# andrewcsmith/vox_box.rs

Hardware: AMD Instinct MI355X
Metric: frames/sec (pitch+LPC+formants), 48 kHz 25 ms/10 ms hop, 1→8 MI355X (higher is better)
Workload: dtype f64

## Files before the change

### vox_box.rs_amd/csrc/k_spectral.hip

```cpp
#include "vbx_spectral_1200.hpp"

namespace vbx {

static size_t spectral_lds_bytes(int n) {
    size_t need = (size_t)pitch_refine_lds_bytes(n);
    const size_t t2_end = (size_t)SP_T2_LDS_OFFSET + 60 * sizeof(double2);
    if (t2_end > need) need = t2_end;
    return (need + 15) & ~(size_t)15;
}

int spectral_plan(int n) {
    static const int min_n = [] { const char *e = getenv("VBX_SPECTRAL_MIN_N"); return e ? atoi(e) : SPECTRAL_MIN_N; }();
    if (n < min_n || n < 64) return SPECTRAL_PLAN_NONE;
    if (n <= 1024) return SPECTRAL_PLAN_1024;
    if (n <= SP_N) return SPECTRAL_PLAN_1200;
    if (n <= 2048) return SPECTRAL_PLAN_2048;
    if (n <= 4096) return SPECTRAL_PLAN_4096;
    return SPECTRAL_PLAN_NONE;
}

int spectral_plan_nc(int plan) {
    return plan == SPECTRAL_PLAN_1200 ? SP_N : plan == SPECTRAL_PLAN_1024 ? 1024 : plan == SPECTRAL_PLAN_2048 ? 2048 :
           plan == SPECTRAL_PLAN_4096 ? 4096 : 0;
}

int spectral_tab_complex(int plan) {
    return plan == SPECTRAL_PLAN_1200 ? SPECTRAL_TAB_COMPLEX : spectral_pow2_tab_complex(plan);
}

void spectral_fill_tab(int plan, double *h) {
    if (plan != SPECTRAL_PLAN_1200) { spectral_pow2_fill_tab(plan, h); return; }
    const long double two_pi = 6.283185307179586476925286766559005768L;
    size_t o = 0;
    auto put = [&](long num, long den) {
        const long double ang = two_pi * (long double)(num % den) / (long double)den;
        h[o++] = (double)cosl(ang); h[o++] = (double)(-sinl(ang));
    };
    for (long np = 0; np < 60; np++) for (long ka = 0; ka < 20; ka++) put(np * ka, 1200);
    for (long c = 0; c < 3; c++) for (long kb = 0; kb < 20; kb++) put(c * kb, 60);
    for (long m = 0; m <= 600; m++) put(m, 2400);
}

bool spectral_supported(int n, int lpc_order, int mfcc_nb, int mfcc_b_lo, int num_coeffs) {
    const int plan = spectral_plan(n);
    if (plan == SPECTRAL_PLAN_NONE) return false;
    if (lpc_order != 0 && lpc_order != SP_LPC_P) return false;
    if (num_coeffs != 0 && ((2 * spectral_plan_nc(plan)) % n != 0 || (n & 1) || num_coeffs > 64 || mfcc_nb < 1 || mfcc_b_lo < 0 || mfcc_b_lo + mfcc_nb > n / 2)) return false;
    return true;
}

int spectral_plan_mfcc(int n) {
    const int plan = spectral_plan(n);
    if (plan == SPECTRAL_PLAN_NONE) return plan;
    if ((2 * spectral_plan_nc(plan)) % n == 0) return plan;
    if (n <= SP_N && (2 * SP_N) % n == 0 && !(n & 1)) return SPECTRAL_PLAN_1200;
    return plan;
}
bool spectral_supported_plan(int plan, int n, int lpc_order, int mfcc_nb, int mfcc_b_lo, int num_coeffs) {
    if (plan == SPECTRAL_PLAN_NONE || n > spectral_plan_nc(plan)) return false;
    if (lpc_order != 0 && lpc_order != SP_LPC_P) return false;
    if (num_coeffs != 0 && ((2 * spectral_plan_nc(plan)) % n != 0 || (n & 1) || num_coeffs > 64 || mfcc_nb < 1 || mfcc_b_lo < 0 || mfcc_b_lo + mfcc_nb > n / 2)) return false;
    return true;
}

static void mfcc_interp_geom(int plan, long *M, int *nt, int *lds_cap) {
    *M = 2L * spectral_plan_nc(plan);
    *nt = plan == SPECTRAL_PLAN_4096 ? 128 : 64;
    *lds_cap = (plan == SPECTRAL_PLAN_1200 || plan == SPECTRAL_PLAN_1024) ? (160 * 1024) / 11 : plan == SPECTRAL_PLAN_2048 ? (160 * 1024) / 7 : (160 * 1024) / 4;
}
static int mfcc_interp_slots(int plan, int nb) { long M; int nt, cap; mfcc_interp_geom(plan, &M, &nt, &cap); return (nb + nt - 1) / nt; }

int mfcc_interp_taps(int plan, int n) {
    long M; int nt, cap; mfcc_interp_geom(plan, &M, &nt, &cap);
    const double tau = 0.5 - (double)n / (2.0 * (double)M);
#ifdef VBX_EXP_INTERP_FEWER_TAPS
    return tau >= 0.36 ? 24 : tau >= 0.268 ? 32 : MFCC_INTERP_MAX_TAPS;
#endif
    return tau >= 0.401 ? 24 : tau >= 0.298 ? 32 : MFCC_INTERP_MAX_TAPS;
}

size_t mfcc_interp_table_bytes(int plan, int nb) {
    long M; int nt, cap; mfcc_interp_geom(plan, &M, &nt, &cap);
    const size_t slots = (size_t)mfcc_interp_slots(plan, nb);
    return (size_t)(M / 4 + 1) * 16 + slots * (MFCC_INTERP_MAX_TAPS / 2) * nt * 16 + slots * nt * 4;
}
size_t mfcc_interp_coef_offset(int plan) { return (size_t)(2L * spectral_plan_nc(plan) / 4 + 1) * 16; }
size_t mfcc_interp_j0_offset(int plan, int nb) {
    long M; int nt, cap; mfcc_interp_geom(plan, &M, &nt, &cap);
    return mfcc_interp_coef_offset(plan) + (size_t)mfcc_interp_slots(plan, nb) * (MFCC_INTERP_MAX_TAPS / 2) * nt * 16;
}

// ... 31 lines not shown
        const long first = (i < nb) ? (k * M) / n - W / 2 + 1 : jmin;
        j0t[i] = (int32_t)(first - jmin);
        for (int t = 0; t < W; t++) {
            long double c = 0.0L;
            if (i < nb) {
                const long num = k * M - (first + t) * (long)n;
                if (num == 0) c = 1.0L;
                else {
                    const long double nu = (long double)num / (long double)n;
                    long r = num % (2L * n); if (r < 0) r += 2L * n;
                    const long double sn = sinl(pi * (long double)r / (long double)n);
                    const long double arg = beta * beta - (2.0L * pi * tau * nu) * (2.0L * pi * tau * nu);
                    const long double bump = sinhc(arg > 0.0L ? sqrtl(arg) : 0.0L) / norm;
                    c = sn / (pi * nu) * bump;
                }
            }
            coef[(((size_t)u * HT + t / 2) * NT + th) * 2 + (t & 1)] = (double)c;
        }
    }
    const int zn = (int)(jmax - jmin + 1), nbp = (nb + 1) & ~1;
    d->jmin = (int)jmin; d->jmax = (int)jmax; d->taps = W;
    d->pu_off = 2 * zn;
    d->lds_bytes = (2 * zn + 2 * nbp + 64) * 8;
    d->rot = nullptr; d->coef = nullptr; d->j0 = nullptr;
    return d->lds_bytes <= cap;
}

bool spectral_list_parked(const spectral_launch_t &L) {
    const bool rows16 = (((uintptr_t)L.out_cand) & 15) == 0 && (L.cand_ld & 1) == 0;
    return L.plan == SPECTRAL_PLAN_1200 && pitch_full_list_bytes(L.n, L.kmax) != 0 && L.kmax >= pitch_full_list_entries(L.n) &&
           L.out_r == nullptr && !L.mfcc_only && rows16;
}

int launch_analyze(hipStream_t s, const spectral_launch_t &L) {
    if (L.x.kind != SAMPLE_F64 && (L.plan != SPECTRAL_PLAN_1200 || L.n != SP_N)) return -1;
    spectral_args_t a;
    a.frames = static_cast<const double *>(L.x.p);
    a.n_frames = L.F; a.stride = L.stride; a.window = L.window; a.lag_window = L.lag_window;
    a.tab = reinterpret_cast<const double2 *>(L.tab);
    a.n = L.n;
    a.pp.sample_rate = L.sample_rate; a.pp.threshold = L.threshold; a.pp.fmin = L.fmin; a.pp.fmax = L.fmax; a.pp.kmax = L.kmax; a.pp.f32 = 0;
    a.out_cand = reinterpret_cast<double *>(L.out_cand); a.cand_ld = L.cand_ld; a.out_count = L.out_count;
    a.pitch_status = L.pitch_status; a.work = L.work;
    a.out_lpc = L.out_lpc; a.lpc_ld = L.lpc_ld;
    a.out_mfcc = L.out_mfcc; a.mfcc_ld = L.mfcc_ld; a.mfcc_status = L.mfcc_status;
    a.bins = L.bins; a.slopes = L.slopes; a.dct = L.dct; a.num_coeffs = L.num_coeffs; a.nb = L.nb;
    a.unsure_list = L.unsure_list; a.unsure_count = L.unsure_count;
    a.out_r = L.out_r; a.n_lags = L.n_lags;
    a.pcm = (L.x.kind == SAMPLE_PCM16 ? SP_FLAG_PCM : 0) | (L.lag_rcp ? SP_FLAG_LAG_RCP : 0) | ((L.mfcc_defer && L.num_coeffs <= 16) ? SP_FLAG_MFCC_DEFER : 0);
    a.mfcc_q = (L.plan != SPECTRAL_PLAN_NONE && L.n > 0) ? (2 * spectral_plan_nc(L.plan)) / L.n : 2;
    a.ip = mfcc_interp_t{};
    if (L.plan != SPECTRAL_PLAN_1200) return launch_analyze_pow2(s, L, a);
    const dim3 grid((unsigned)L.F), block(64);
    const size_t base = spectral_lds_bytes(L.n);
    size_t extra = pitch_full_list_bytes(L.n, L.kmax);
    a.pp.full_off = extra ? (int)base : 0;
    if (spectral_list_parked(L)) { a.pp.full_off = -1; extra = 0; }
    const size_t lds = base + extra;
    const bool lpc = L.out_lpc != nullptr, mf = L.out_mfcc != nullptr;
    if (L.mfcc_only) {
        if (L.interp && L.n != SP_N) {
            a.ip = L.ip;
            const size_t li = spectral_lds_bytes(0) > (size_t)L.ip.lds_bytes ? spectral_lds_bytes(0) : (((size_t)L.ip.lds_bytes + 15) & ~(size_t)15);
            hipLaunchKernelGGL((analyze_kernel<false, true, false, SP_MFCC_ONLY_INTERP>), grid, block, li, s, a);
        } else hipLaunchKernelGGL((analyze_kernel<false, true, true, SP_MFCC_ONLY>), grid, block, spectral_lds_bytes(0), s, a);
        return 0;
    }
    if (L.out_r != nullptr) {
        if (L.n == SP_N) hipLaunchKernelGGL((analyze_kernel<false, false, true, SP_AC_ONLY>), grid, block, spectral_lds_bytes(0), s, a);
        else hipLaunchKernelGGL((analyze_kernel<false, false, false, SP_AC_ONLY>), grid, block, spectral_lds_bytes(0), s, a);
        return 0;
    }
    static const bool want3 = [] { const char *e = getenv("VBX_SPECTRAL_W3"); return e == nullptr || atoi(e) != 0; }();
    const bool w3 = want3 && extra == 0 && 12 * lds <= 160 * 1024;
    if (L.x.kind == SAMPLE_F32) {
        launch_analyze_f32in(s, a, (unsigned)L.F, lds, lpc, mf, w3);
        return 0;
    }
#define VBX_SP_LAUNCH(LPC_, MF_, FULL_)                                                                              \
    do {                                                                                                              \
        if (w3) hipLaunchKernelGGL((analyze_kernel<LPC_, MF_, FULL_, SP_ANALYZE, 3>), grid, block, lds, s, a);        \
        else hipLaunchKernelGGL((analyze_kernel<LPC_, MF_, FULL_>), grid, block, lds, s, a);                          \
    } while (0)
    if (L.interp && mf && L.n != SP_N) {
        a.ip = L.ip;
        const size_t li = lds > (size_t)L.ip.lds_bytes ? lds : (((size_t)L.ip.lds_bytes + 15) & ~(size_t)15);
        const bool w3i = want3 && extra == 0 && 12 * li <= 160 * 1024;
        if (lpc) { if (w3i) hipLaunchKernelGGL((analyze_kernel<true, true, false, SP_ANALYZE_INTERP, 3>), grid, block, li, s, a);
                   else hipLaunchKernelGGL((analyze_kernel<true, true, false, SP_ANALYZE_INTERP>), grid, block, li, s, a); }
        else { if (w3i) hipLaunchKernelGGL((analyze_kernel<false, true, false, SP_ANALYZE_INTERP, 3>), grid, block, li, s, a);
               else hipLaunchKernelGGL((analyze_kernel<false, true, false, SP_ANALYZE_INTERP>), grid, block, li, s, a); }
    } else if (L.n != SP_N) {
        if (lpc && mf) VBX_SP_LAUNCH(true, true, false);
        else if (mf) VBX_SP_LAUNCH(false, true, false);
        else if (lpc) VBX_SP_LAUNCH(true, false, false);
        else VBX_SP_LAUNCH(false, false, false);
    } else if (lpc && mf) VBX_SP_LAUNCH(true, true, true);
    else if (lpc) VBX_SP_LAUNCH(true, false, true);
    else if (mf) VBX_SP_LAUNCH(false, true, true);
    else VBX_SP_LAUNCH(false, false, true);
#undef VBX_SP_LAUNCH
    return 0;
}

}
```

### vox_box.rs_amd/csrc/vbx_api.hip

```cpp
#include "vbx_ctx.hpp"

#include <cmath>
#include <cstdio>
#include <cstdlib>
#include <cstring>
#include <dlfcn.h>
#include <string>
#include <vector>

using namespace vbx;

extern "C" const double VBX_MALE_FORMANT_ESTIMATES[4] = {320., 1440., 2760., 3200.};
extern "C" const double VBX_FEMALE_FORMANT_ESTIMATES[4] = {480., 1760., 3200., 3520.};

namespace {

thread_local std::string g_last_error;

}

namespace vbx {

int fail(vbx_ctx *ctx, int code, const std::string &msg) {
    g_last_error = msg;
// ... 1009 lines not shown
                          const int64_t *h_seg_start, size_t n_segments,
                          const vbx_resonance *h_est_init, size_t n_est,
                          vbx_resonance *out_formants, vbx_resonance *out_res, int32_t *out_res_count,
                          double *out_coeffs, int32_t *status) {
    int rc = check_frames(ctx, __func__, x, n_frames, frame_len, stride, VBX_MAX_LONG_FRAME_LEN);
    if (rc != VBX_SUCCESS) return rc < 0 ? rc : VBX_SUCCESS;
    VBX_HIP(ctx, hipSetDevice(ctx->device));
    return run_find_formants(ctx, ctx->stream, x, n_frames, frame_len, stride, sample_rate, n_coeffs, h_seg_start, n_segments,
                             h_est_init, n_est, out_formants, 2 * n_est, out_res, out_res_count, out_coeffs, status);
}

int vbx_internal_track_stitch(vbx_ctx *ctx, void *stream, vbx_resonance *formants, size_t n_frames, size_t formants_ld,
                              size_t first, size_t stop, const double *d_state_in, int32_t *d_changed) {
    VBX_REQUIRE(ctx, ctx != nullptr, "null context");
    VBX_REQUIRE(ctx, formants && d_state_in, "null argument");
    const auto &lt = ctx->last_track;
    VBX_REQUIRE(ctx, lt.res != nullptr && lt.out == (res_t *)formants && lt.F == (long)n_frames && lt.out_ld == (long)formants_ld,
                "the formant rows are not the ones the last find_formants / analyze_frames call on this context wrote");
    VBX_REQUIRE(ctx, first <= stop && stop <= n_frames, "need first <= stop <= n_frames");
    VBX_HIP(ctx, hipSetDevice(ctx->device));
    hipStream_t st = stream ? (hipStream_t)stream : ctx->stream;
    { Prof p(ctx, "tracker_stitch", st);
      launch_tracker_stitch(st, lt.res, lt.F, VBX_MAX_RESONANCES, lt.cnt, lt.n_est, lt.st, lt.out, lt.out_ld, (long)first, (long)stop,
                            d_state_in, d_changed); }
    return check_launch(ctx, "vbx_track_stitch_f64");
}

int vbx_track_stitch_f64(vbx_ctx *ctx, vbx_resonance *formants, size_t n_frames, size_t formants_ld, size_t first, size_t stop,
                         const vbx_resonance *d_state_in, int32_t *d_changed) {
    return vbx_internal_track_stitch(ctx, nullptr, formants, n_frames, formants_ld, first, stop, (const double *)d_state_in, d_changed);
}

int vbx_internal_last_spectral_split(vbx_ctx *ctx) { return ctx ? ctx->last_spectral_split : 0; }
int vbx_internal_last_mfcc_interp(vbx_ctx *ctx) { return ctx ? ctx->last_mfcc_interp : 0; }
int vbx_internal_last_mfcc_form(vbx_ctx *ctx) { return ctx ? ctx->last_mfcc_form : 0; }
int vbx_internal_last_pitch_form(vbx_ctx *ctx) { return ctx ? ctx->last_pitch_form : 0; }

int vbx_internal_mfcc_interp_table(size_t frame_len, int b_lo, int nb, int32_t *desc, void *buf, size_t cap, size_t *need) {
    if (!desc || !need || frame_len < 2 || frame_len > VBX_MAX_FRAME_LEN || nb < 1 || nb > 4096) return VBX_E_INVALID;
    const int plan = spectral_plan_mfcc((int)frame_len);
    if (plan == SPECTRAL_PLAN_NONE || (2 * spectral_plan_nc(plan)) % (int)frame_len == 0) return 0;
    const size_t bytes = mfcc_interp_table_bytes(plan, nb);
    *need = bytes;
    std::vector<char> h(bytes, 0);
    mfcc_interp_t d{};
    if (!mfcc_interp_fill(plan, (int)frame_len, b_lo, nb, h.data(), &d)) return 0;
    const int nt = plan == SPECTRAL_PLAN_4096 ? 128 : 64;
    desc[0] = 4 * spectral_plan_nc(plan) / 2; desc[1] = nt; desc[2] = (nb + nt - 1) / nt; desc[3] = d.taps;
    desc[4] = d.jmin; desc[5] = d.jmax; desc[6] = (int32_t)mfcc_interp_coef_offset(plan); desc[7] = (int32_t)mfcc_interp_j0_offset(plan, nb);
    if (buf && cap >= bytes) std::memcpy(buf, h.data(), bytes);
    return 1;
}

int vbx_internal_mfcc_table_plans(size_t frame_len, int b_lo, int nb, int32_t *out) {
    if (!out || frame_len < 2 || frame_len > VBX_MAX_FRAME_LEN || b_lo < 0 || nb < 1 || nb > 4096) return VBX_E_INVALID;
    const mfcc_mplan_t m = mfcc_mfma_plan((int)frame_len, b_lo, nb);
    const mfcc_plan_t p = mfcc_plan((int)frame_len, nb);
    const int32_t v[14] = {m.ok, m.n1, m.n2, m.k2, m.mt, m.ntd, m.ntm, m.src0, m.src1, p.ok, p.n1, p.n2, p.nc, p.tm};
    std::memcpy(out, v, sizeof v);
    return VBX_SUCCESS;
}


}

namespace vbx {

int run_mfcc(vbx_ctx *ctx, hipStream_t stm, const double *x, size_t n_frames, size_t frame_len, size_t stride,
             const double *window, size_t num_coeffs, double lo_hz, double hi_hz,
             double sample_rate, double *out, size_t out_ld, int32_t *status) {
    VBX_REQUIRE(ctx, out != nullptr, "null output");
    VBX_REQUIRE(ctx, num_coeffs >= 1 && num_coeffs <= 64, "num_coeffs must be in [1, 64]");
    VBX_REQUIRE(ctx, out_ld >= num_coeffs, "output rows must hold num_coeffs entries");
    std::vector<int32_t> hb; bool bad = false; const int32_t *d_bins = nullptr;
    ctx->last_mfcc_interp = 0;
    ctx->last_mfcc_form = 0;
    int rc = get_bins_dev(ctx, frame_len, num_coeffs, lo_hz, hi_hz, sample_rate, &d_bins, hb, bad);
    if (rc != VBX_SUCCESS) return rc;
    if (bad) {
        ctx->last_mfcc_form = 8;
        { Prof p(ctx, "fill_rows", stm); launch_fill_rows(stm, out, (long)n_frames, (int)num_coeffs, (long)out_ld, 0.0, status, VBX_FRAME_ERR_PANIC); }
        return check_launch(ctx, "vbx_mfcc_f64");
    }
    const int nb = hb.back() - hb.front();
    const double *dct = nullptr, *slopes = nullptr;
    VBX_HIP(ctx, ctx->tables.dct(num_coeffs, &dct));
    VBX_HIP(ctx, ctx->tables.slopes(frame_len, num_coeffs, lo_hz, hi_hz, sample_rate, hb, &slopes));
    if (frame_len > VBX_MAX_FRAME_LEN) {
        VBX_REQUIRE(ctx, nb >= 1, "no mel bins");
        const double *tw = nullptr;
        VBX_HIP(ctx, ctx->tables.goertzel(frame_len, hb.front(), nb, &tw));
        void *w = nullptr;
        rc = ws_get(ctx, vbx_ctx::WS_CZT, mfcc_long_scratch_bytes((long)n_frames, nb), &w); if (rc != VBX_SUCCESS) return rc;
        ctx->last_mfcc_form = 7;
        { Prof p(ctx, "mfcc_long", stm);
          launch_mfcc_long(stm, x, (long)n_frames, (long)frame_len, (long)stride, window, tw, d_bins, slopes, dct, (int)num_coeffs, nb, out,
                           (long)out_ld, status, (double *)w); }
        return check_launch(ctx, "vbx_mfcc_f64");
    }
    {
        int plan = spectral_plan((int)frame_len);
        if (frame_len == 2048) plan = SPECTRAL_PLAN_1024; else if (frame_len == 4096) plan = SPECTRAL_PLAN_2048;
        if (!ctx->mfcc_force_goertzel && !ctx->mfcc_force_dft2 && !ctx->mfcc_force_mfma && plan != SPECTRAL_PLAN_NONE &&
            ((int)frame_len == spectral_plan_nc(plan) || (int)frame_len == 2 * spectral_plan_nc(plan)) &&
            num_coeffs <= 64 && nb >= 1 && hb.front() >= 0 && hb.front() + nb <= (int)frame_len / 2) {
            const double *tab = nullptr;
// ... 263 lines not shown
```

### vox_box.rs_amd/csrc/vbx_kernels.hpp

```cpp
#pragma once

#include <hip/hip_runtime.h>
#include <stdint.h>

#define VBX_MAX_LPC_ORDER_K 62
#define VBX_MAX_FRAME_LEN_K 4096
#define VBX_MAX_RESONANCES_K 32
#define VBX_FORMANT_SLOTS_K 6

namespace vbx {

struct frame_map_t { long seg_len, t0, tc; };
__host__ __device__ inline long frame_map(const frame_map_t &m, long i, long n_frames) {
    if (m.seg_len == 0) return (i < n_frames) ? i : -1;
    const long t = m.t0 + i % m.tc, f = (i / m.tc) * m.seg_len + t;
    return (t < m.seg_len && t < m.t0 + m.tc && f < n_frames) ? f : -1;
}
inline long frame_map_items(const frame_map_t &m, long n_frames) {
    return m.seg_len == 0 ? n_frames : ((n_frames + m.seg_len - 1) / m.seg_len) * m.tc;
}


struct res_t { double frequency, bandwidth; };
struct pitch_t { double frequency, strength; };
// ... 67 lines not shown
bool formant_resonances_fast_supported(int p);
void launch_formant_resonances_fast(hipStream_t s, const double *coeffs, long F, int p, double sample_rate,
                                    res_t *out_res, int32_t *out_count, int32_t *status, frame_map_t map, int32_t *redo_count);

void launch_tracker(hipStream_t s, const res_t *res, long F, int n_res, const int32_t *res_count,
                    const int64_t *seg_start, long n_seg, const res_t *est_init, int n_est,
                    const int32_t *frame_status, res_t *out, long out_ld ,
                    long t0 = 0 , long tc = 0x7fffffffffffffffL );

size_t tracker_chunked_workspace_bytes(long F);
void launch_tracker_chunked(hipStream_t s, const res_t *res, long F, int n_res, const int32_t *res_count,
                            const int64_t *seg_start, long n_seg, const res_t *est_init, int n_est,
                            const int32_t *frame_status, res_t *out, long out_ld, void *ws);

void launch_tracker_stitch(hipStream_t s, const res_t *res, long F, int n_res, const int32_t *res_count, int n_est,
                           const int32_t *frame_status, res_t *out, long out_ld, long first, long stop,
                           const double *state_in , int32_t *changed );

size_t pitch_lds_bytes(int n);
constexpr int PITCH_LIST_LANES = 64;
size_t pitch_full_list_bytes(int n, int kmax);
constexpr int PITCH_WORK_SLOTS = 64;
constexpr int PHASE_SLOTS = 16;
constexpr int PITCH_WORK_WORDS = PITCH_WORK_SLOTS * 4 + PITCH_WORK_SLOTS * PHASE_SLOTS;
#ifdef VBX_EXP_PHASES
#define VBX_PHASE_INIT() unsigned long long _tp = __builtin_readcyclecounter()
#define VBX_PHASE(work_, f_, k_)                                                                                   \
    do {                                                                                                            \
        asm volatile("s_waitcnt vmcnt(0) lgkmcnt(0)" ::: "memory");                                                 \
        const unsigned long long _t = __builtin_readcyclecounter();                                                 \
        if ((work_) != nullptr && lane_id() == 0)                                                                   \
            atomicAdd((work_) + PITCH_WORK_SLOTS * 4 + ((f_) & (PITCH_WORK_SLOTS - 1)) * PHASE_SLOTS + (k_), _t - _tp); \
        _tp = _t;                                                                                                   \
    } while (0)
#else
#define VBX_PHASE_INIT() do { } while (0)
#define VBX_PHASE(work_, f_, k_) do { } while (0)
#endif
void launch_pitch(hipStream_t s, const double *x, long F, int n, long stride, const double *window,
                  const double *lag_window, double sample_rate, double threshold, double fmin, double fmax,
                  int kmax, pitch_t *out_cand, long cand_ld ,
                  int32_t *out_count, int32_t *status, unsigned long long *work);
void launch_pitch_list(hipStream_t s, const int32_t *frame_list, const int32_t *list_count, int grid, frames_t x, int n, long stride,
                       const double *window, const double *lag_window, double sample_rate, double threshold, double fmin, double fmax,
                       int kmax, pitch_t *out_cand, long cand_ld, int32_t *out_count, int32_t *status, unsigned long long *work);
void launch_sinc_points(hipStream_t s, const double *y, int ylen, long offset, long nx, const double *xs, long m,
                        long depth, double *out, int32_t *status);
void launch_extremum_points(hipStream_t s, const double *y, int ylen, long offset, long nx, const double *ix, long m,
                            long depth, double *out_xy, int32_t *status, int interp = 2 ,
                            int is_max = 1);

constexpr int SPECTRAL_N = 1200;
constexpr int SPECTRAL_LPC_ORDER = 12;
constexpr int SPECTRAL_TAB_COMPLEX = 60 * 20 + 3 * 20 + 601;
enum { SPECTRAL_PLAN_NONE = 0, SPECTRAL_PLAN_1200 = 1, SPECTRAL_PLAN_1024 = 2, SPECTRAL_PLAN_2048 = 3, SPECTRAL_PLAN_4096 = 4,
       SPECTRAL_PLANS = 5 };
constexpr int SPECTRAL_AC_MIN_LAGS = 64;
constexpr int SPECTRAL_MIN_N = 512;
int spectral_plan(int n);
int spectral_plan_mfcc(int n);
bool spectral_supported_plan(int plan, int n, int lpc_order, int mfcc_nb, int mfcc_b_lo, int num_coeffs);
int spectral_plan_nc(int plan);
int spectral_tab_complex(int plan);
void spectral_fill_tab(int plan, double *h_out);
int spectral_pow2_tab_complex(int plan);
void spectral_pow2_fill_tab(int plan, double *h_out);
constexpr int MFCC_INTERP_MAX_TAPS = 40;
struct mfcc_interp_t {
    const double *rot;
    const double *coef;
    const int32_t *j0;
    int jmin, jmax;
    int taps;
    int pu_off;
    int lds_bytes;
};
int mfcc_interp_taps(int plan, int n);
size_t mfcc_interp_table_bytes(int plan, int nb);
size_t mfcc_interp_coef_offset(int plan);
size_t mfcc_interp_j0_offset(int plan, int nb);
bool mfcc_interp_fill(int plan, int n, int b_lo, int nb, void *h_table, mfcc_interp_t *h_desc );

struct spectral_launch_t {
    int plan; int n;
    frames_t x;
    long F; long stride; const double *window; const double *lag_window; const double *tab;
    bool mfcc_defer;
    bool lag_rcp;
    double sample_rate, threshold, fmin, fmax; int kmax;
    pitch_t *out_cand; long cand_ld; int32_t *out_count; int32_t *pitch_status; unsigned long long *work;
    double *out_lpc; long lpc_ld;
    double *out_mfcc; long mfcc_ld; int32_t *mfcc_status;
    const int32_t *bins; const double *slopes; const double *dct; int num_coeffs; int nb;
    int32_t *unsure_list; int32_t *unsure_count;
    int32_t *lpc_list; int32_t *lpc_count;
    bool mfcc_only;
    double *out_r; int n_lags;
    bool whole_curve;
    bool interp; mfcc_interp_t ip;
    double *curve_ws; size_t curve_ws_bytes;
};
size_t spectral_split_row_bytes(int n, double sample_rate, double fmin);
bool spectral_supported(int n, int lpc_order, int mfcc_nb, int mfcc_b_lo, int num_coeffs);
bool spectral_list_parked(const spectral_launch_t &L);
int launch_analyze(hipStream_t s, const spectral_launch_t &L);
void launch_mfcc_rows(hipStream_t s, double *rows, long F, long ld, int num_coeffs, const double *dct);
bool lpc_exact_supported(int n, int p);
// ... 232 lines not shown
```

### vox_box.rs_amd/csrc/vbx_spectral_1200.hpp

```cpp
#pragma once

#include <type_traits>
#include "vbx_device.hpp"
#include "vbx_kernels.hpp"
#include "vbx_mfcc_tail.hpp"
#include "vbx_mfcc_interp.hpp"
#include "vbx_pitch_refine.hpp"
#include "vbx_spectral.hpp"

namespace vbx {

constexpr int SP_N = SPECTRAL_N;
constexpr int SP_M = 2 * SP_N;
constexpr int SP_S1 = 61;
constexpr int SP_S2 = 404;
constexpr int SP_T1 = 0;
constexpr int SP_T2 = SP_T1 + 60 * 20;
constexpr int SP_TM = SP_T2 + 3 * 20;
static_assert(SP_TM + 601 == SPECTRAL_TAB_COMPLEX, "table layout");
constexpr int SP_T2_LDS_OFFSET = (2 * 602 + 64) * 8;
static_assert(SP_T2_LDS_OFFSET >= (20 * SP_S1 > 3 * SP_S2 ? 20 * SP_S1 : 3 * SP_S2) * 8 && SP_T2_LDS_OFFSET % 16 == 0, "T2 behind both");

__device__ __forceinline__ void dft5(double &r0, double &i0, double &r1, double &i1, double &r2, double &i2,
                                     double &r3, double &i3, double &r4, double &i4) {
    constexpr double C5 = 0.55901699437494742410;
    constexpr double S1 = 0.95105651629515357212;
    constexpr double S2 = 0.58778525229247312917;
    const double t1r = r1 + r4, t1i = i1 + i4, t3r = r1 - r4, t3i = i1 - i4;
    const double t2r = r2 + r3, t2i = i2 + i3, t4r = r2 - r3, t4i = i2 - i3;
    const double t5r = t1r + t2r, t5i = t1i + t2i;
    const double m1r = fma(-0.25, t5r, r0), m1i = fma(-0.25, t5i, i0);
    const double m2r = C5 * (t1r - t2r), m2i = C5 * (t1i - t2i);
    const double s1r = m1r + m2r, s1i = m1i + m2i, s2r = m1r - m2r, s2i = m1i - m2i;
    const double ur = fma(S1, t3r, S2 * t4r), ui = fma(S1, t3i, S2 * t4i);
    const double vr = fma(S2, t3r, -(S1 * t4r)), vi = fma(S2, t3i, -(S1 * t4i));
    r0 = r0 + t5r; i0 = i0 + t5i;
    r1 = s1r + ui; i1 = s1i - ur;
    r4 = s1r - ui; i4 = s1i + ur;
    r2 = s2r + vi; i2 = s2i - vr;
    r3 = s2r - vi; i3 = s2i + vr;
}

__host__ __device__ constexpr int dft20_in(int n1, int n2) { return (5 * n1 + 4 * n2) % 20; }
__host__ __device__ constexpr int dft20_slot(int k) { return (5 * (k % 4) + 4 * (k % 5)) % 20; }

__device__ __forceinline__ void dft20(double (&re)[20], double (&im)[20]) {
#pragma unroll
    for (int n2 = 0; n2 < 5; n2++)
        dft4(re[dft20_in(0, n2)], im[dft20_in(0, n2)], re[dft20_in(1, n2)], im[dft20_in(1, n2)],
             re[dft20_in(2, n2)], im[dft20_in(2, n2)], re[dft20_in(3, n2)], im[dft20_in(3, n2)]);
#pragma unroll
    for (int k1 = 0; k1 < 4; k1++)
        dft5(re[dft20_in(k1, 0)], im[dft20_in(k1, 0)], re[dft20_in(k1, 1)], im[dft20_in(k1, 1)],
             re[dft20_in(k1, 2)], im[dft20_in(k1, 2)], re[dft20_in(k1, 3)], im[dft20_in(k1, 3)],
             re[dft20_in(k1, 4)], im[dft20_in(k1, 4)]);
}

#ifndef VBX_EXP_TWB
#define VBX_EXP_TWB 2
#endif
constexpr int TWB = VBX_EXP_TWB;
#ifndef VBX_EXP_MB1
#define VBX_EXP_MB1 3
#endif
template <int TWB = vbx::TWB>
__device__ __forceinline__ void twiddle_tight(double (&re)[20], double (&im)[20], const double2 *tw_row) {
#pragma unroll
    for (int h = 0; h < 20 / TWB; h++) {
        double2 tw[TWB];
#pragma unroll
        for (int k = 0; k < TWB; k++) tw[k] = tw_row[TWB * h + k];
#pragma unroll
        for (int k = 0; k < TWB; k++) {
            if (TWB * h + k == 0) continue;
            const int s = dft20_slot(TWB * h + k);
            const double a = re[s], b = im[s];
            re[s] = fma(a, tw[k].x, -(b * tw[k].y));
            im[s] = fma(a, tw[k].y, b * tw[k].x);
            asm volatile("" : "+v"(re[s]), "+v"(im[s]));
        }
        asm volatile("" ::: "memory");
    }
}

template <int KC, bool TIGHT = false>
__device__ __forceinline__ void fft1200(double (&re)[20], double (&im)[20], double (&xr)[7][3], double (&xi)[7][3],
                                        double *ex, const double2 *tab, const double2 *t2) {
    const int lane = lane_id();
    const int np = (lane < 60) ? lane : 59;
    const bool act = lane < 60;
    dft20(re, im);
    if constexpr (TIGHT) twiddle_tight(re, im, tab + SP_T1 + np * 20);
    else {
#pragma unroll
    for (int h = 0; h < 2; h++) {
        double2 tw[10];
#pragma unroll
        for (int k = 0; k < 10; k++) tw[k] = tab[SP_T1 + np * 20 + 10 * h + k];
#pragma unroll
        for (int k = 0; k < 10; k++) {
            if (10 * h + k == 0) continue;
            const int s = dft20_slot(10 * h + k);
            const double a = re[s], b = im[s];
            re[s] = fma(a, tw[k].x, -(b * tw[k].y));
            im[s] = fma(a, tw[k].y, b * tw[k].x);
        }
    }
    }
    const int ka2 = np % 20, c2 = np / 20;
    double br[20], bi[20];
    wave_sync();
#pragma unroll
    for (int k = 0; k < 20; k++) if (act) ex[k * SP_S1 + lane] = re[dft20_slot(k)];
    wave_sync();
#pragma unroll
    for (int b = 0; b < 20; b++) br[b] = ex[ka2 * SP_S1 + 3 * b + c2];
    wave_sync();
#pragma unroll
    for (int k = 0; k < 20; k++) if (act) ex[k * SP_S1 + lane] = im[dft20_slot(k)];
    wave_sync();
#pragma unroll
    for (int b = 0; b < 20; b++) bi[b] = ex[ka2 * SP_S1 + 3 * b + c2];
    dft20(br, bi);
    if constexpr (TIGHT) twiddle_tight<4>(br, bi, t2 + c2 * 20);
    else {
#pragma unroll
    for (int h = 0; h < 2; h++) {
        double2 tw[10];
#pragma unroll
        for (int k = 0; k < 10; k++) tw[k] = t2[c2 * 20 + 10 * h + k];
#pragma unroll
        for (int k = 0; k < 10; k++) {
            if (10 * h + k == 0) continue;
            const int s = dft20_slot(10 * h + k);
            const double a = br[s], b = bi[s];
            br[s] = fma(a, tw[k].x, -(b * tw[k].y));
            bi[s] = fma(a, tw[k].y, b * tw[k].x);
        }
    }
    }
    double vr[7][3], vi[7][3];
    wave_sync();
#pragma unroll
    for (int k = 0; k < 20; k++) if (act) ex[c2 * SP_S2 + ka2 + 20 * k] = br[dft20_slot(k)];
    wave_sync();
#pragma unroll
    for (int t = 0; t < 7; t++)
#pragma unroll
        for (int c = 0; c < 3; c++) vr[t][c] = (t < 6 || lane < 16) ? ex[c * SP_S2 + lane + 64 * t] : 0.0;
    wave_sync();
#pragma unroll
    for (int k = 0; k < 20; k++) if (act) ex[c2 * SP_S2 + ka2 + 20 * k] = bi[dft20_slot(k)];
    wave_sync();
#pragma unroll
    for (int t = 0; t < 7; t++)
#pragma unroll
        for (int c = 0; c < 3; c++) vi[t][c] = (t < 6 || lane < 16) ? ex[c * SP_S2 + lane + 64 * t] : 0.0;
    wave_sync();
    constexpr double H3 = 0.86602540378443864676;
#pragma unroll
    for (int t = 0; t < 7; t++) {
        const double sr = vr[t][1] + vr[t][2], si = vi[t][1] + vi[t][2];
        const double dr = vr[t][1] - vr[t][2], di = vi[t][1] - vi[t][2];
        xr[t][0] = vr[t][0] + sr; xi[t][0] = vi[t][0] + si;
        const double mr = fma(-0.5, sr, vr[t][0]), mi = fma(-0.5, si, vi[t][0]);
        xr[t][1] = fma(H3, di, mr); xi[t][1] = fma(-H3, dr, mi);
        if (KC == 3) { xr[t][2] = fma(-H3, di, mr); xi[t][2] = fma(H3, dr, mi); }
        else { xr[t][2] = 0.0; xi[t][2] = 0.0; }
    }
}

#ifndef VBX_SPECTRAL_WAVES
#define VBX_SPECTRAL_WAVES 2
#endif
#ifndef VBX_EXP_CELL_NB
#define VBX_EXP_CELL_NB 3
#endif
#ifndef VBX_EXP_CELL_NB_F32IN
#define VBX_EXP_CELL_NB_F32IN VBX_EXP_CELL_NB
#endif
#ifndef VBX_EXP_FRONT_END_ONCE
#define VBX_EXP_FRONT_END_ONCE 1
#endif
__host__ __device__ constexpr bool sp_front_end_once(bool mfcc, bool full, int waves, bool f32) {
    return VBX_EXP_FRONT_END_ONCE != 0 && !(!mfcc && full && waves >= 3 && !f32);
}
__host__ __device__ constexpr int sp_cell_blocks(int waves, bool f32) { return f32 ? VBX_EXP_CELL_NB_F32IN : VBX_EXP_CELL_NB; }
template <bool LPC, bool MFCC, bool FULL, int MODE = SP_ANALYZE, int WAVES = VBX_SPECTRAL_WAVES, typename TIN = double>
__global__ __launch_bounds__(64) __attribute__((amdgpu_waves_per_eu(sp_is_mfcc_only(MODE) ? 2 : WAVES, sp_is_mfcc_only(MODE) ? 4 : WAVES))) void analyze_kernel(const spectral_args_t a) {
    constexpr bool F32 = std::is_same<TIN, float>::value;
    static_assert(!F32 || (FULL && MODE == SP_ANALYZE), "float samples: the fused analysis of full frames");
    static_assert(MODE != SP_MFCC_ONLY || (MFCC && FULL && !LPC), "the MFCC-only form needs the full frame and has no lag sums");
    static_assert(MODE != SP_AC_ONLY || (!MFCC && !LPC), "the autocorrelation-only form");
    static_assert(!sp_is_interp(MODE) || (MFCC && !FULL), "interpolated bins: a padded frame's MFCC");
    static_assert(MODE != SP_MFCC_ONLY_INTERP || !LPC, "the MFCC-only forms have no lag sums");
    constexpr bool PITCH = !sp_is_mfcc_only(MODE);
    constexpr bool INTERP = sp_is_interp(MODE);
    extern __shared__ __attribute__((aligned(16))) double smem[];
    const long f = xcd_item(blockIdx.x, a.n_frames);
    if (f >= a.n_frames) return;
    const int lane = lane_id();
    const int np = (lane < 60) ? lane : 59;
    const int n = FULL ? SP_N : a.n;
    double *ex = smem;
    const double *xf = a.frames + f * a.stride;
    double2 *t2 = reinterpret_cast<double2 *>(reinterpret_cast<char *>(smem) + SP_T2_LDS_OFFSET);
    VBX_PHASE_INIT();

    double re[20], im[20];
    const int16_t *x16 = reinterpret_cast<const int16_t *>(a.frames) + f * a.stride;
    const float *x32 = reinterpret_cast<const float *>(a.frames) + f * a.stride;
    {
        const bool al = ((((uintptr_t)xf) | ((uintptr_t)a.window)) & 15) == 0;
        double2 xv[10], wv[10];
        float2 xs32[F32 ? 10 : 1];
#pragma unroll
        for (int q = 0; q < 10; q++) {
            const int i = 120 * q + 2 * np;
            if constexpr (F32) {
                float lo, hi;
                if ((((uintptr_t)x32) & 7) == 0) { const float2 w = *reinterpret_cast<const float2 *>(x32 + i); lo = w.x; hi = w.y; }
                else { lo = x32[i]; hi = x32[i + 1]; }
                xs32[q] = float2{lo, hi};
                wv[q] = (a.window != nullptr) ? (((uintptr_t)a.window & 15) == 0 ? *reinterpret_cast<const double2 *>(a.window + i)
                                                                                  : double2{a.window[i], a.window[i + 1]}) : double2{1.0, 1.0};
            } else if (FULL && (a.pcm & SP_FLAG_PCM)) {
                int lo, hi;
                if ((((uintptr_t)x16) & 3) == 0) { const int w = *reinterpret_cast<const int *>(x16 + i); lo = (short)(w & 0xffff); hi = w >> 16; }
                else { lo = x16[i]; hi = x16[i + 1]; }
                xv[q] = double2{pcm16_value(lo), pcm16_value(hi)};
                wv[q] = (a.window != nullptr) ? (((uintptr_t)a.window & 15) == 0 ? *reinterpret_cast<const double2 *>(a.window + i)
                                                                                  : double2{a.window[i], a.window[i + 1]}) : double2{1.0, 1.0};
            } else if (al && i + 1 < n) {
                xv[q] = *reinterpret_cast<const double2 *>(xf + i);
                wv[q] = (a.window != nullptr) ? *reinterpret_cast<const double2 *>(a.window + i) : double2{1.0, 1.0};
            } else {
                xv[q] = double2{0.0, 0.0}; wv[q] = double2{1.0, 1.0};
                if (i < n) { xv[q].x = xf[i]; if (a.window != nullptr) wv[q].x = a.window[i]; }
                if (i + 1 < n) { xv[q].y = xf[i + 1]; if (a.window != nullptr) wv[q].y = a.window[i + 1]; }
            }
        }
#pragma unroll
        for (int q = 0; q < 10; q++) {
            if constexpr (F32) xv[q] = double2{(double)xs32[q].x, (double)xs32[q].y};
            re[q] = (a.window != nullptr) ? xv[q].x * wv[q].x : xv[q].x;
            im[q] = (a.window != nullptr) ? xv[q].y * wv[q].y : xv[q].y;
        }
#pragma unroll
        for (int q = 10; q < 20; q++) { re[q] = 0.0; im[q] = 0.0; }
    }
    const double x0 = readlane_f64(re[0], 0);
    if (lane < 60) t2[lane] = a.tab[SP_T2 + lane];
    VBX_PHASE(a.work, f, 0);

    double xr[7][3], xi[7][3];
    fft1200<3, (WAVES >= 3)>(re, im, xr, xi, ex, a.tab, t2);
    VBX_PHASE(a.work, f, 1);

    double ar[10], ai[10], br[10], bi[10];
#pragma unroll
    for (int t = 0; t < 7; t++)
#pragma unroll
        for (int kc = 0; kc < 3; kc++) if (t < 6 || lane < 16) ex[lane + 64 * t + 400 * kc] = xr[t][kc];
    wave_sync();
#pragma unroll
    for (int t = 0; t < 10; t++) {
        const int m = lane + 64 * t;
        const bool ok = m <= 600;
        ar[t] = ok ? ex[m] : 0.0;
        br[t] = ok ? ex[(m == 0) ? 0 : SP_N - m] : 0.0;
    }
    wave_sync();
#pragma unroll
    for (int t = 0; t < 7; t++)
#pragma unroll
        for (int kc = 0; kc < 3; kc++) if (t < 6 || lane < 16) ex[lane + 64 * t + 400 * kc] = xi[t][kc];
    wave_sync();
#pragma unroll
    for (int t = 0; t < 10; t++) {
        const int m = lane + 64 * t;
        const bool ok = m <= 600;
        ai[t] = ok ? ex[m] : 0.0;
        bi[t] = ok ? ex[(m == 0) ? 0 : SP_N - m] : 0.0;
    }
    wave_sync();

    const int b_lo = MFCC ? a.bins[0] : 0;
    double pk[10], pn[10];
    double2 *zc = reinterpret_cast<double2 *>(ex);
    double2 rot_m = double2{1.0, 0.0}, rot_step = double2{1.0, 0.0};
    if constexpr (INTERP) { rot_m = reinterpret_cast<const double2 *>(a.ip.rot)[lane]; rot_step = reinterpret_cast<const double2 *>(a.ip.rot)[64]; }
#pragma unroll
    for (int t = 0; t < 10; t++) {
        const int m = lane + 64 * t;
        const double2 w = a.tab[SP_TM + ((m <= 600) ? m : 0)];
        const double er = 0.5 * (ar[t] + br[t]), ei = 0.5 * (ai[t] - bi[t]);
        const double o_r = 0.5 * (ai[t] + bi[t]), o_i = -0.5 * (ar[t] - br[t]);
        const double tr = fma(w.x, o_r, -(w.y * o_i)), ti = fma(w.x, o_i, w.y * o_r);
        const double pr = er + tr, pi = ei + ti, qr = er - tr, qi = ei - ti;
        pk[t] = fma(pr, pr, pi * pi);
        pn[t] = fma(qr, qr, qi * qi);
        if constexpr (INTERP) {
            asm volatile("" : "+v"(pk[t]), "+v"(pn[t]));
            mfcc_interp_stage(zc, a.ip, m, pr, pi, rot_m, rot_step, t == 0);
        }
    }

    if constexpr (INTERP) {
        wave_sync();
// ... 81 lines not shown
                    const int b1 = (FULL ? (m >> 1) : m / q) - b_lo;
                    c1[u] = (on && b1 >= 0 && b1 < a.nb) ? b1 : -1;
                    s1[u] = *reinterpret_cast<const double2 *>(a.slopes + 2 * (c1[u] < 0 ? 0 : c1[u]));
                }
#pragma unroll
                for (int u = 0; u < MB1; u++) {
                    const int t = MB1 * h + u;
                    if (t < 10 && c1[u] >= 0) {
                        pu[c1[u]] = fabs(pk[t]) * s1[u].x;
                        pd[c1[u]] = fabs(sqrt(pk[t])) * s1[u].y;
                    }
                }
            }
        } else
#pragma unroll
        for (int h = 0; h < 10 / MB; h++) {
            double2 s1[MB], s2[MB];
            int c1[MB], c2[MB];
#pragma unroll
            for (int u = 0; u < MB; u++) {
                const int t = MB * h + u, m = lane + 64 * t;
                const bool on = m <= 600 && (FULL ? (m & 1) == 0 : m % q == 0);
                const int mq = FULL ? (m >> 1) : m / q;
                const int b1 = mq - b_lo, b2 = (half - mq) - b_lo;
                c1[u] = (on && b1 >= 0 && b1 < a.nb) ? b1 : -1;
                c2[u] = (on && b2 >= 0 && b2 < a.nb && b2 != b1) ? b2 : -1;
                s1[u] = *reinterpret_cast<const double2 *>(a.slopes + 2 * (c1[u] < 0 ? 0 : c1[u]));
                s2[u] = *reinterpret_cast<const double2 *>(a.slopes + 2 * (c2[u] < 0 ? 0 : c2[u]));
            }
#pragma unroll
            for (int u = 0; u < MB; u++) {
                const int t = MB * h + u;
                if (c1[u] >= 0) {
                    pu[c1[u]] = fabs(pk[t]) * s1[u].x;
                    pd[c1[u]] = fabs(sqrt(pk[t])) * s1[u].y;
                }
                if (c2[u] >= 0) {
                    pu[c2[u]] = fabs(pn[t]) * s2[u].x;
                    pd[c2[u]] = fabs(sqrt(pn[t])) * s2[u].y;
                }
            }
        }
        wave_sync();
        VBX_PHASE(a.work, f, 13);
        if (a.num_coeffs <= 16) mfcc_tail_q(pu, pd, en, a.bins, a.dct, a.num_coeffs, b_lo, lane, a.out_mfcc + f * a.mfcc_ld, a.work, f, (a.pcm & SP_FLAG_MFCC_DEFER) != 0);
        else mfcc_tail_m(pu, pd, en, a.bins, a.dct, a.num_coeffs, b_lo, lane, a.out_mfcc + f * a.mfcc_ld);
        if (a.mfcc_status != nullptr && lane == 0) a.mfcc_status[f] = 0;
        wave_sync();
    }

    VBX_PHASE(a.work, f, 3);
    if constexpr (!PITCH) return;

    fft1200<2, (WAVES >= 3)>(re, im, xr, xi, ex, a.tab, t2);
    VBX_PHASE(a.work, f, 4);

    constexpr double INV_M = 1.0 / (double)SP_M;
    double r_e[11], r_o[11];
    int jj[11];
#pragma unroll
    for (int s = 0; s < 11; s++) {
        const int t = (s < 7) ? s : s - 7, kc = (s < 7) ? 0 : 1;
        const int q = lane + 64 * t;
        const bool ok = (kc == 0) ? (q < 400) : (q < 200);
        jj[s] = ok ? q + 400 * kc : -1;
        r_e[s] = xr[t][kc] * INV_M;
        r_o[s] = -(xi[t][kc] * INV_M);
    }
    const double s0 = readlane_f64(r_e[0], 0);
    if (x0 != 0.0) {
#pragma unroll
        for (int s = 0; s < 11; s++) {
            const int i = 2 * jj[s];
            if (jj[s] >= 0 && i < n) {
                const double xs = F32 ? (double)x32[i] : (FULL && (a.pcm & SP_FLAG_PCM)) ? pcm16_value(x16[i]) : xf[i];
                const double xe = (a.window != nullptr) ? xs * a.window[i] : xs;
                r_e[s] = (r_e[s] - x0 * xe) + x0;
            }
            if (jj[s] >= 0 && i + 1 < n) {
                const double xs = F32 ? (double)x32[i + 1] : (FULL && (a.pcm & SP_FLAG_PCM)) ? pcm16_value(x16[i + 1]) : xf[i + 1];
                const double xo = (a.window != nullptr) ? xs * a.window[i + 1] : xs;
                r_o[s] = (r_o[s] - x0 * xo) + x0;
            }
        }
    }
    if constexpr (MODE == SP_AC_ONLY) {
        double *row = a.out_r + f * (long)a.n_lags;
        const bool al = ((((uintptr_t)a.out_r) & 15) == 0) && (a.n_lags & 1) == 0;
#pragma unroll
        for (int s = 0; s < 11; s++) {
            const int i = 2 * jj[s];
            if (jj[s] >= 0 && i + 1 < a.n_lags && al) *reinterpret_cast<double2 *>(row + i) = double2{r_e[s], r_o[s]};
            else {
                if (jj[s] >= 0 && i < a.n_lags) row[i] = r_e[s];
                if (jj[s] >= 0 && i + 1 < a.n_lags) row[i + 1] = r_o[s];
            }
        }
        return;
    }
    if (LPC) {
        static_assert(SP_LPC_P == 12, "seven lanes hold r[0..12]");
        double *row = a.out_lpc + f * a.lpc_ld;
        if (lane < 7) { row[2 * lane] = r_e[0]; if (lane < 6) row[2 * lane + 1] = r_o[0]; }
    }
    double amax = -1.0;
#pragma unroll
    for (int s = 0; s < 11; s++) {
// ... 81 lines not shown
```

Before: 40.20 million.

## Stream FFT-1200 twiddles into LDS via async global_load_lds with lane-major table

```diff
diff --git a/vox_box.rs_amd/csrc/k_spectral.hip b/vox_box.rs_amd/csrc/k_spectral.hip
--- a/vox_box.rs_amd/csrc/k_spectral.hip
+++ b/vox_box.rs_amd/csrc/k_spectral.hip
@@ -2,9 +2,10 @@
 
 namespace vbx {
 
-static size_t spectral_lds_bytes(int n) {
+static size_t spectral_lds_bytes(int n, bool stream = false) {
     size_t need = (size_t)pitch_refine_lds_bytes(n);
-    const size_t t2_end = (size_t)SP_T2_LDS_OFFSET + 60 * sizeof(double2);
+    const size_t t2_end = stream ? (size_t)SP_TW_LDS_END
+                                 : (size_t)SP_T2_LDS_OFFSET + 60 * sizeof(double2);
     if (t2_end > need) need = t2_end;
     return (need + 15) & ~(size_t)15;
 }
@@ -36,7 +37,7 @@
         const long double ang = two_pi * (long double)(num % den) / (long double)den;
         h[o++] = (double)cosl(ang); h[o++] = (double)(-sinl(ang));
     };
-    for (long np = 0; np < 60; np++) for (long ka = 0; ka < 20; ka++) put(np * ka, 1200);
+    for (long ka = 0; ka < 20; ka++) for (long lane = 0; lane < 64; lane++) put((lane < 60 ? lane : 59) * ka, 1200);
     for (long c = 0; c < 3; c++) for (long kb = 0; kb < 20; kb++) put(c * kb, 60);
     for (long m = 0; m <= 600; m++) put(m, 2400);
 }
@@ -174,8 +175,11 @@
     a.ip = mfcc_interp_t{};
     if (L.plan != SPECTRAL_PLAN_1200) return launch_analyze_pow2(s, L, a);
     const dim3 grid((unsigned)L.F), block(64);
-    const size_t base = spectral_lds_bytes(L.n);
+    static const bool want3 = [] { const char *e = getenv("VBX_SPECTRAL_W3"); return e == nullptr || atoi(e) != 0; }();
     size_t extra = pitch_full_list_bytes(L.n, L.kmax);
+    const bool w3_form = want3 && !L.mfcc_only && L.out_r == nullptr && (extra == 0 || spectral_list_parked(L));
+    const size_t base = spectral_lds_bytes(L.n, VBX_EXP_TW_STREAM != 0 && w3_form);
+    static_assert(12 * SP_TW_LDS_END <= 160 * 1024, "the streamed form keeps twelve frames per CU");
     a.pp.full_off = extra ? (int)base : 0;
     if (spectral_list_parked(L)) { a.pp.full_off = -1; extra = 0; }
     const size_t lds = base + extra;
@@ -193,7 +197,6 @@
         else hipLaunchKernelGGL((analyze_kernel<false, false, false, SP_AC_ONLY>), grid, block, spectral_lds_bytes(0), s, a);
         return 0;
     }
-    static const bool want3 = [] { const char *e = getenv("VBX_SPECTRAL_W3"); return e == nullptr || atoi(e) != 0; }();
     const bool w3 = want3 && extra == 0 && 12 * lds <= 160 * 1024;
     if (L.x.kind == SAMPLE_F32) {
         launch_analyze_f32in(s, a, (unsigned)L.F, lds, lpc, mf, w3);
diff --git a/vox_box.rs_amd/csrc/vbx_api.hip b/vox_box.rs_amd/csrc/vbx_api.hip
--- a/vox_box.rs_amd/csrc/vbx_api.hip
+++ b/vox_box.rs_amd/csrc/vbx_api.hip
@@ -1085,6 +1085,14 @@
     return 1;
 }
 
+int vbx_internal_spectral_table(int plan, double *buf, size_t cap, size_t *need) {
+    if (!need) return VBX_E_INVALID;
+    if (plan <= SPECTRAL_PLAN_NONE || plan >= SPECTRAL_PLANS) return 0;
+    *need = 2 * (size_t)spectral_tab_complex(plan);
+    if (buf && cap >= *need) spectral_fill_tab(plan, buf);
+    return 1;
+}
+
 int vbx_internal_mfcc_table_plans(size_t frame_len, int b_lo, int nb, int32_t *out) {
     if (!out || frame_len < 2 || frame_len > VBX_MAX_FRAME_LEN || b_lo < 0 || nb < 1 || nb > 4096) return VBX_E_INVALID;
     const mfcc_mplan_t m = mfcc_mfma_plan((int)frame_len, b_lo, nb);
diff --git a/vox_box.rs_amd/csrc/vbx_kernels.hpp b/vox_box.rs_amd/csrc/vbx_kernels.hpp
--- a/vox_box.rs_amd/csrc/vbx_kernels.hpp
+++ b/vox_box.rs_amd/csrc/vbx_kernels.hpp
@@ -143,7 +143,7 @@
 
 constexpr int SPECTRAL_N = 1200;
 constexpr int SPECTRAL_LPC_ORDER = 12;
-constexpr int SPECTRAL_TAB_COMPLEX = 60 * 20 + 3 * 20 + 601;
+constexpr int SPECTRAL_TAB_COMPLEX = 20 * 64 + 3 * 20 + 601;
 enum { SPECTRAL_PLAN_NONE = 0, SPECTRAL_PLAN_1200 = 1, SPECTRAL_PLAN_1024 = 2, SPECTRAL_PLAN_2048 = 3, SPECTRAL_PLAN_4096 = 4,
        SPECTRAL_PLANS = 5 };
 constexpr int SPECTRAL_AC_MIN_LAGS = 64;
diff --git a/vox_box.rs_amd/csrc/vbx_spectral_1200.hpp b/vox_box.rs_amd/csrc/vbx_spectral_1200.hpp
--- a/vox_box.rs_amd/csrc/vbx_spectral_1200.hpp
+++ b/vox_box.rs_amd/csrc/vbx_spectral_1200.hpp
@@ -15,11 +15,23 @@
 constexpr int SP_S1 = 61;
 constexpr int SP_S2 = 404;
 constexpr int SP_T1 = 0;
-constexpr int SP_T2 = SP_T1 + 60 * 20;
+constexpr int SP_T2 = SP_T1 + 20 * 64;
 constexpr int SP_TM = SP_T2 + 3 * 20;
 static_assert(SP_TM + 601 == SPECTRAL_TAB_COMPLEX, "table layout");
 constexpr int SP_T2_LDS_OFFSET = (2 * 602 + 64) * 8;
 static_assert(SP_T2_LDS_OFFSET >= (20 * SP_S1 > 3 * SP_S2 ? 20 * SP_S1 : 3 * SP_S2) * 8 && SP_T2_LDS_OFFSET % 16 == 0, "T2 behind both");
+constexpr int SP_T2_LDS_BYTES = 1024;
+constexpr int SP_TW_SLOT_BYTES = 64 * 16;
+constexpr int SP_TW_SLOTS_EX = 9, SP_TW_SLOTS = 11;
+__host__ __device__ constexpr int sp_tw_slot_offset(int slot) {
+    return slot < SP_TW_SLOTS_EX ? slot * SP_TW_SLOT_BYTES : SP_T2_LDS_OFFSET + SP_T2_LDS_BYTES + (slot - SP_TW_SLOTS_EX) * SP_TW_SLOT_BYTES;
+}
+__host__ __device__ constexpr int sp_tw_slot_of(int ka) { return (ka - 1) % SP_TW_SLOTS; }
+constexpr int SP_TW_LDS_END = sp_tw_slot_offset(SP_TW_SLOTS - 1) + SP_TW_SLOT_BYTES;
+static_assert(SP_TW_SLOTS_EX * SP_TW_SLOT_BYTES <= 20 * SP_S1 * 8, "slots 0..8 inside the exchange buffer");
+static_assert(SP_TW_SLOTS_EX * SP_TW_SLOT_BYTES <= SP_T2_LDS_OFFSET && 60 * 16 <= SP_T2_LDS_BYTES, "no slot over the T2 copy");
+static_assert(sp_tw_slot_offset(SP_TW_SLOTS_EX) == SP_T2_LDS_OFFSET + SP_T2_LDS_BYTES, "slots 9, 10 right behind the T2 copy");
+static_assert(SP_TW_LDS_END <= pitch_refine_lds_bytes(SP_N) && pitch_refine_lds_bytes(SP_N) == 13512, "the full frame's LDS does not grow");
 
 __device__ __forceinline__ void dft5(double &r0, double &i0, double &r1, double &i1, double &r2, double &i2,
                                      double &r3, double &i3, double &r4, double &i4) {
@@ -63,13 +75,13 @@
 #ifndef VBX_EXP_MB1
 #define VBX_EXP_MB1 3
 #endif
-template <int TWB = vbx::TWB>
+template <int TWB = vbx::TWB, int LD = 1>
 __device__ __forceinline__ void twiddle_tight(double (&re)[20], double (&im)[20], const double2 *tw_row) {
 #pragma unroll
     for (int h = 0; h < 20 / TWB; h++) {
         double2 tw[TWB];
 #pragma unroll
-        for (int k = 0; k < TWB; k++) tw[k] = tw_row[TWB * h + k];
+        for (int k = 0; k < TWB; k++) tw[k] = tw_row[LD * (TWB * h + k)];
 #pragma unroll
         for (int k = 0; k < TWB; k++) {
             if (TWB * h + k == 0) continue;
@@ -83,20 +95,89 @@
     }
 }
 
-template <int KC, bool TIGHT = false>
+__device__ __forceinline__ void tw_load_lds(const double2 *src, double *smem, int lds_bytes) {
+    __builtin_amdgcn_global_load_lds((const __attribute__((address_space(1))) void *)src,
+                                     (__attribute__((address_space(3))) void *)(reinterpret_cast<char *>(smem) + lds_bytes), 16, 0, 0);
+}
+template <int LEFT>
+__device__ __forceinline__ void tw_stream_wait() {
+    asm volatile("s_waitcnt vmcnt(%0)" :: "n"(LEFT) : "memory");
+}
+__device__ __forceinline__ const double2 *tw_lane_column(const double2 *tab, int lane) {
+    const double2 *p = tab + lane;
+    asm volatile("" : "+v"(p));
+    return p;
+}
+template <bool WITH_T2>
+__device__ __forceinline__ void tw_stream_round(const double2 *tab, double *smem, int lane) {
+    asm volatile("s_waitcnt lgkmcnt(0)" ::: "memory");
+    const double2 *col = tw_lane_column(tab, lane);
+    if constexpr (WITH_T2) tw_load_lds(col + SP_T2, smem, SP_T2_LDS_OFFSET);
+#pragma unroll
+    for (int ka = 1; ka <= SP_TW_SLOTS; ka++) tw_load_lds(col + SP_T1 + ka * 64, smem, sp_tw_slot_offset(sp_tw_slot_of(ka)));
+}
+typedef double tw_pair_t __attribute__((ext_vector_type(2)));
+template <int H>
+__device__ __forceinline__ void tw_stream_batch(double (&re)[20], double (&im)[20], const double2 *tab, double *smem, int lane, unsigned mine) {
+    if constexpr (H == 3) tw_stream_wait<4>();
+    if constexpr (H == 4) tw_stream_wait<0>();
+    tw_pair_t tw[4];
+    constexpr int K0 = (H == 0) ? 1 : 0;
+    constexpr int O1 = sp_tw_slot_offset(sp_tw_slot_of(4 * H + 1)), O2 = sp_tw_slot_offset(sp_tw_slot_of(4 * H + 2)),
+                  O3 = sp_tw_slot_offset(sp_tw_slot_of(4 * H + 3));
+    if constexpr (H == 0)
+        asm volatile("ds_read_b128 %0, %3 offset:%4\n\tds_read_b128 %1, %3 offset:%5\n\tds_read_b128 %2, %3 offset:%6\n\ts_waitcnt lgkmcnt(0)"
+                     : "=&v"(tw[1]), "=&v"(tw[2]), "=&v"(tw[3]) : "v"(mine), "n"(O1), "n"(O2), "n"(O3) : "memory");
+    else {
+        constexpr int O0 = sp_tw_slot_offset(sp_tw_slot_of(4 * H));
+        asm volatile("ds_read_b128 %0, %4 offset:%5\n\tds_read_b128 %1, %4 offset:%6\n\tds_read_b128 %2, %4 offset:%7\n\t"
+                     "ds_read_b128 %3, %4 offset:%8\n\ts_waitcnt lgkmcnt(0)"
+                     : "=&v"(tw[0]), "=&v"(tw[1]), "=&v"(tw[2]), "=&v"(tw[3]) : "v"(mine), "n"(O0), "n"(O1), "n"(O2), "n"(O3) : "memory");
+    }
+#pragma unroll
+    for (int k = K0; k < 4; k++) {
+        const int s = dft20_slot(4 * H + k);
+        const double a = re[s], b = im[s];
+        re[s] = fma(a, tw[k].x, -(b * tw[k].y));
+        im[s] = fma(a, tw[k].y, b * tw[k].x);
+        asm volatile("" : "+v"(re[s]), "+v"(im[s]));
+    }
+    asm volatile("" ::: "memory");
+    if constexpr (4 * H + K0 + SP_TW_SLOTS < 20) {
+        const double2 *col = tw_lane_column(tab, lane);
+#pragma unroll
+        for (int k = K0; k < 4; k++) {
+            const int ka = 4 * H + k + SP_TW_SLOTS;
+            if (ka < 20) tw_load_lds(col + SP_T1 + ka * 64, smem, sp_tw_slot_offset(sp_tw_slot_of(ka)));
+        }
+    }
+}
+__device__ __forceinline__ void tw_stream_products(double (&re)[20], double (&im)[20], const double2 *tab, double *smem, int lane) {
+    unsigned mine = (unsigned)(unsigned long)(__attribute__((address_space(3))) char *)(reinterpret_cast<char *>(smem));
+    asm volatile("v_lshl_add_u32 %0, %1, 4, %0" : "+v"(mine) : "v"(lane));
+    tw_stream_wait<0>();
+    tw_stream_batch<0>(re, im, tab, smem, lane, mine);
+    tw_stream_batch<1>(re, im, tab, smem, lane, mine);
+    tw_stream_batch<2>(re, im, tab, smem, lane, mine);
+    tw_stream_batch<3>(re, im, tab, smem, lane, mine);
+    tw_stream_batch<4>(re, im, tab, smem, lane, mine);
+}
+
+template <int KC, bool TIGHT = false, bool STREAM = false>
 __device__ __forceinline__ void fft1200(double (&re)[20], double (&im)[20], double (&xr)[7][3], double (&xi)[7][3],
                                         double *ex, const double2 *tab, const double2 *t2) {
     const int lane = lane_id();
     const int np = (lane < 60) ? lane : 59;
     const bool act = lane < 60;
     dft20(re, im);
-    if constexpr (TIGHT) twiddle_tight(re, im, tab + SP_T1 + np * 20);
+    if constexpr (TIGHT && STREAM) tw_stream_products(re, im, tab, ex, lane);
+    else if constexpr (TIGHT) twiddle_tight<TWB, 64>(re, im, tab + SP_T1 + np);
     else {
 #pragma unroll
     for (int h = 0; h < 2; h++) {
         double2 tw[10];
 #pragma unroll
-        for (int k = 0; k < 10; k++) tw[k] = tab[SP_T1 + np * 20 + 10 * h + k];
+        for (int k = 0; k < 10; k++) tw[k] = tab[SP_T1 + (10 * h + k) * 64 + np];
 #pragma unroll
         for (int k = 0; k < 10; k++) {
             if (10 * h + k == 0) continue;
@@ -186,6 +267,10 @@
     return VBX_EXP_FRONT_END_ONCE != 0 && !(!mfcc && full && waves >= 3 && !f32);
 }
 __host__ __device__ constexpr int sp_cell_blocks(int waves, bool f32) { return f32 ? VBX_EXP_CELL_NB_F32IN : VBX_EXP_CELL_NB; }
+#ifndef VBX_EXP_TW_STREAM
+#define VBX_EXP_TW_STREAM 1
+#endif
+__host__ __device__ constexpr bool sp_tw_stream(int waves) { return VBX_EXP_TW_STREAM != 0 && waves >= 3; }
 template <bool LPC, bool MFCC, bool FULL, int MODE = SP_ANALYZE, int WAVES = VBX_SPECTRAL_WAVES, typename TIN = double>
 __global__ __launch_bounds__(64) __attribute__((amdgpu_waves_per_eu(sp_is_mfcc_only(MODE) ? 2 : WAVES, sp_is_mfcc_only(MODE) ? 4 : WAVES))) void analyze_kernel(const spectral_args_t a) {
     constexpr bool F32 = std::is_same<TIN, float>::value;
@@ -206,7 +291,8 @@
     const double *xf = a.frames + f * a.stride;
     double2 *t2 = reinterpret_cast<double2 *>(reinterpret_cast<char *>(smem) + SP_T2_LDS_OFFSET);
     VBX_PHASE_INIT();
-
+    constexpr bool TIGHT = WAVES >= 3;
+    constexpr bool STREAM = sp_tw_stream(WAVES);
     double re[20], im[20];
     const int16_t *x16 = reinterpret_cast<const int16_t *>(a.frames) + f * a.stride;
     const float *x32 = reinterpret_cast<const float *>(a.frames) + f * a.stride;
@@ -250,11 +336,12 @@
         for (int q = 10; q < 20; q++) { re[q] = 0.0; im[q] = 0.0; }
     }
     const double x0 = readlane_f64(re[0], 0);
-    if (lane < 60) t2[lane] = a.tab[SP_T2 + lane];
+    if constexpr (STREAM) tw_stream_round<true>(a.tab, smem, lane);
+    else if (lane < 60) t2[lane] = a.tab[SP_T2 + lane];
     VBX_PHASE(a.work, f, 0);
 
     double xr[7][3], xi[7][3];
-    fft1200<3, (WAVES >= 3)>(re, im, xr, xi, ex, a.tab, t2);
+    fft1200<3, TIGHT, STREAM>(re, im, xr, xi, ex, a.tab, t2);
     VBX_PHASE(a.work, f, 1);
 
     double ar[10], ai[10], br[10], bi[10];
@@ -442,7 +529,8 @@
     VBX_PHASE(a.work, f, 3);
     if constexpr (!PITCH) return;
 
-    fft1200<2, (WAVES >= 3)>(re, im, xr, xi, ex, a.tab, t2);
+    if constexpr (STREAM) tw_stream_round<false>(a.tab, smem, lane);
+    fft1200<2, TIGHT, STREAM>(re, im, xr, xi, ex, a.tab, t2);
     VBX_PHASE(a.work, f, 4);
 
     constexpr double INV_M = 1.0 / (double)SP_M;
```

After: 40.38 million (median of 6 runs). Within noise of the previous version (+0.5%).
